# AlexIoannides/bodywork-mlops-demo

Measured on NVIDIA H100. Metric: train rows/sec (N x 128 least-squares fit), higher is better.
Workload: dtype bf16x2 (hi+lo) MMA operands, f32 accumulate, f64 fold+solve

## Files before the change

### bodywork-mlops-demo_b200/csrc/b2_api.cu

```cuda
#include <dlfcn.h>
#include <math.h>
#include <stdarg.h>
#include <stdlib.h>

#include <new>
#include <thread>
#include <vector>

#include "b2_internal.cuh"
#include "b2_xchg.cuh"

namespace b2 {

static thread_local char g_err[768] = "";

void set_error(const char* fmt, ...) {
  va_list ap;
  va_start(ap, fmt);
  vsnprintf(g_err, sizeof(g_err), fmt, ap);
  va_end(ap);
}

namespace {

// ... 242 lines not shown
      },
      [&](int buf, int64_t, int64_t rows) {
        return gram_dispatch(ctx, ctx->stage_x[buf], x_dtype, ctx->stage_y[buf], rows, d, d,
                             mask != nullptr ? ctx->stage_m[buf] : nullptr, keep);
      });
}

int ensure_s_cleared(b2_ctx* ctx) {
  if (ctx->s_zero_pending) {
    B2_CUDA(cudaMemsetAsync(ctx->S, 0, sizeof(double) * kMaxS * kMaxS, ctx->stream));
    ctx->s_zero_pending = false;
  }
  return B2_OK;
}

}

}

using namespace b2;

extern "C" {

int b2_abi_version(void) { return B2_ABI_VERSION; }
const char* b2_last_error(void) { return g_err; }

int b2_device_count(int* n_out) {
  if (n_out == nullptr) { set_error("n_out is null"); return B2_E_ARG; }
  int n = 0;
  cudaError_t e = cudaGetDeviceCount(&n);
  if (e != cudaSuccess) {
    cudaGetLastError();
    *n_out = 0;
    set_error("cudaGetDeviceCount: %s", cudaGetErrorString(e));
    return B2_E_CUDA;
  }
  *n_out = n;
  return B2_OK;
}

static int ctx_allocate(b2_ctx* ctx) {
  B2_CUDA(cudaStreamCreateWithFlags(&ctx->stream, cudaStreamNonBlocking));
  B2_CUDA(cudaStreamCreateWithFlags(&ctx->copy_stream, cudaStreamNonBlocking));
  B2_CUDA(cudaEventCreate(&ctx->ev_t0));
  B2_CUDA(cudaEventCreate(&ctx->ev_t1));
  for (int i = 0; i < kKernelEventPairs; ++i) {
    B2_CUDA(cudaEventCreate(&ctx->ev_k[i][0]));
    B2_CUDA(cudaEventCreate(&ctx->ev_k[i][1]));
  }
  ctx->simt_ctas = ctx->sm_count;
  ctx->score_ctas = ctx->sm_count * 8;
  B2_CUDA(cudaMalloc(reinterpret_cast<void**>(&ctx->S), sizeof(double) * kMaxS * kMaxS));
  B2_CUDA(cudaMalloc(reinterpret_cast<void**>(&ctx->tc_part),
                     sizeof(double) * (size_t)ctx->sm_count * (kTcAccElems + kTcSums)));
  B2_CUDA(cudaMalloc(reinterpret_cast<void**>(&ctx->tc_red), sizeof(double) * (kTcAccElems + 16)));
  B2_CUDA(cudaMalloc(reinterpret_cast<void**>(&ctx->shift), gram_shift_bytes()));
  B2_CUDA(cudaMalloc(reinterpret_cast<void**>(&ctx->simt_part), sizeof(double) * (size_t)ctx->simt_ctas * kMaxS * kMaxS));
  B2_CUDA(cudaMalloc(reinterpret_cast<void**>(&ctx->score_part), sizeof(double) * ((size_t)ctx->score_ctas + 2) * kNStats));
  B2_CUDA(cudaMalloc(reinterpret_cast<void**>(&ctx->coef_dev), sizeof(double) * (kMaxD + 1)));
  B2_CUDA(cudaMalloc(reinterpret_cast<void**>(&ctx->grad_part), sizeof(double) * (size_t)ctx->score_ctas * kGradOut));
  B2_CUDA(cudaMalloc(reinterpret_cast<void**>(&ctx->refine), sizeof(double) * kRfDoubles));
  B2_CUDA(cudaMalloc(reinterpret_cast<void**>(&ctx->loo), sizeof(double) * kLooDoubles));
  B2_CUDA(cudaMalloc(reinterpret_cast<void**>(&ctx->loo_part), sizeof(double) * (size_t)ctx->sm_count * kMaxAlphas));
  B2_CUDA(cudaMalloc(reinterpret_cast<void**>(&ctx->solve_out), sizeof(double) * (2 * kMaxD + 8)));
  B2_CUDA(cudaHostAlloc(reinterpret_cast<void**>(&ctx->solve_host), sizeof(double) * (2 * kMaxD + 8), cudaHostAllocDefault));
  B2_CUDA(cudaMalloc(reinterpret_cast<void**>(&ctx->tc_sync), 64));
  B2_CUDA(cudaMemset(ctx->tc_sync, 0, 64));
  B2_CUDA(cudaHostAlloc(reinterpret_cast<void**>(&ctx->xchg_status_host), 64, cudaHostAllocDefault));
  ctx->xchg_status_host[0] = 0u;
  B2_CUDA(cudaHostAlloc(reinterpret_cast<void**>(&ctx->coef_host), 2 * sizeof(double) * (kMaxD + 1), cudaHostAllocDefault));
  for (int b = 0; b < 2; ++b) B2_CUDA(cudaEventCreateWithFlags(&ctx->ev_coef[b], cudaEventDisableTiming));
  B2_CUDA(cudaMemset(ctx->shift, 0, gram_shift_bytes()));
  B2_CUDA(cudaMemset(ctx->S, 0, sizeof(double) * kMaxS * kMaxS));
  B2_CUDA(cudaMemset(ctx->tc_red, 0, sizeof(double) * (kTcAccElems + 16)));
  return B2_OK;
}

int b2_ctx_create(int device, b2_ctx** out) {
  if (out == nullptr) { set_error("out is null"); return B2_E_ARG; }
  *out = nullptr;
  int n = 0;
  if (b2_device_count(&n) != B2_OK || n == 0) {
    set_error("no usable CUDA device (libb2gram has no CPU fallback)");
    return B2_E_CUDA;
  }
  if (device < 0 || device >= n) { set_error("device %d out of range (0..%d)", device, n - 1); return B2_E_ARG; }
  B2_CUDA(cudaSetDevice(device));
  cudaDeviceProp prop;
  B2_CUDA(cudaGetDeviceProperties(&prop, device));
  if (prop.major != 9 || prop.minor != 0) {
    set_error("device %d is sm_%d%d; libb2gram is built for sm_90a (H100) only", device, prop.major, prop.minor);
    return B2_E_UNSUPPORTED;
  }
  b2_ctx* ctx = new (std::nothrow) b2_ctx();
  if (ctx == nullptr) { set_error("out of host memory"); return B2_E_STATE; }
  ctx->device = device;
  ctx->sm_count = prop.multiProcessorCount;
  ctx->hbm_bytes = prop.totalGlobalMem;
  snprintf(ctx->name, sizeof(ctx->name), "%s", prop.name);
  if (int r = ctx_allocate(ctx)) {
    b2_ctx_destroy(ctx);
    return r;
  }
  *out = ctx;
  return B2_OK;
}

// ... 1157 lines not shown
```

### bodywork-mlops-demo_b200/csrc/b2_internal.cuh

```cuda
#pragma once
#include <cuda.h>
#include <cuda_bf16.h>
#include <cuda_runtime.h>
#include <stdint.h>
#include <stdio.h>
#include <string.h>

#include <type_traits>

#include "../../include/b2gram.h"

namespace b2 {

constexpr int kMaxD = B2_MAX_D;
constexpr int kMaxS = kMaxD + 2;
constexpr int kKernelEventPairs = 64;
constexpr int kMaxRanks = 8;
constexpr size_t kXchgSlotDoubles = (size_t)kMaxS * kMaxS;
constexpr size_t kXchgDataDoubles = 2 * kMaxRanks * kXchgSlotDoubles;
constexpr size_t kXchgBytes = kXchgDataDoubles * sizeof(double) + 256;

constexpr int kTcRows = 64;
constexpr int kTcM = 128;
constexpr int kTcEMax = 16;
inline int tc_e_width(int pack) { return pack >= 3 ? 16 : 8; }
constexpr int kTcTri = kTcM * (kTcM + 1) / 2;
__host__ __device__ constexpr int tc_part_index(int acc, int i, int j, int ew) {
  return acc == 0 ? (j < kTcM ? j * (j + 1) / 2 + i : kTcTri + (j - kTcM) * kTcM + i)
                  : kTcTri + ew * kTcM + j * kTcM + i;
}
__host__ __device__ constexpr int tc_part_elems(int ew, bool d2) {
  return kTcTri + ew * kTcM + (d2 ? (kTcM + ew) * kTcM : 0);
}
constexpr int kTcAccElems = tc_part_elems(kTcEMax, true);
constexpr int kTcSums = 3;

constexpr int kNStats = 10;
constexpr int kGradOut = kMaxD + 1;
constexpr int kRfBeta = 0;
constexpr int kRfB0 = kMaxD;
constexpr int kRfMean = kMaxD + 1;
constexpr int kRfPrevBeta = 2 * kMaxD + 1;
constexpr int kRfPrevB0 = 3 * kMaxD + 1;
constexpr int kRfStep = 3 * kMaxD + 2;
constexpr int kRfGrad = 3 * kMaxD + 3;
constexpr int kRfDoubles = kRfGrad + kGradOut;
constexpr int kOutRefineStep = 2 * kMaxD + 3;
constexpr int kOutRefineGuard = 2 * kMaxD + 4;

constexpr int kMaxAlphas = B2_MAX_ALPHAS;
constexpr int kLooQ = 0;
constexpr int kLooLam = kMaxD * kMaxD;
constexpr int kLooMean = kLooLam + kMaxD;
constexpr int kLooC = kLooMean + kMaxD;
constexpr int kLooMisc = kLooC + kMaxD;
constexpr int kLooAlpha = kLooMisc + 8;
constexpr int kLooCw = kLooAlpha + kMaxAlphas;
constexpr int kLooW = kLooCw + kMaxD * kMaxAlphas;
constexpr int kLooSum = kLooW + kMaxD * kMaxAlphas;
constexpr int kLooDoubles = kLooSum + kMaxAlphas;

struct EnetArgs {
  double l1_ratio, eps, tol;
  int n_alphas, grid, max_iter, positive, fit_intercept;
  double* alphas;
  const double* coef_init;
  double *coefs, *intercepts, *gaps, *iters, *tol_out;
  const double* folds = nullptr;
  const double* l1_ratios = nullptr;
  int n_folds = 1, n_l1 = 1;
  double* mse = nullptr;
};

constexpr int kMaxFolds = 254;
int launch_fold_ranges(b2_ctx* ctx, const uint8_t* fold_of_row, int64_t n, int n_folds, unsigned long long* range);
int launch_fold_sum(b2_ctx* ctx, const double* folds, int n_folds, int d, double* S);

inline int narrow_dp(int d) { return d <= 1 ? 1 : d <= 2 ? 2 : d <= 4 ? 4 : d <= 8 ? 8 : 16; }

void set_error(const char* fmt, ...);

#define B2_CUDA(call)                                                                      \
  do {                                                                                     \
    cudaError_t e_ = (call);                                                               \
    if (e_ != cudaSuccess) {                                                               \
      b2::set_error("%s failed: %s (%s:%d)", #call, cudaGetErrorString(e_), __FILE__, __LINE__); \
      return B2_E_CUDA;                                                                    \
    }                                                                                      \
  } while (0)

}

struct b2_ctx {
  int device = 0;
  int sm_count = 0;
  size_t hbm_bytes = 0;
  char name[128] = {0};
  cudaStream_t stream = nullptr;
  cudaStream_t copy_stream = nullptr;
  cudaEvent_t ev_t0 = nullptr, ev_t1 = nullptr;
  cudaEvent_t ev_k[b2::kKernelEventPairs][2];
  int k_pairs = 0;
  int64_t launches = 0;

  int kernel_mode = B2_KERNEL_AUTO;
  int drain_rows = 8192;
  int precision = B2_PRECISION_SPLIT;

  int d = 0;
  double* S = nullptr;

  double* tc_part = nullptr;
  double* tc_red = nullptr;
  float* shift = nullptr;
  bool solve_attr_set = false;
  double* solve_host = nullptr;
  struct TmCache {
    const void* X = nullptr; const float* y = nullptr; const uint8_t* mask = nullptr;
    int64_t n = 0, ldx = 0; int d = 0, x_dtype = -1;
    int y_map_2d = 0, m_map_2d = 0;
    alignas(64) unsigned char tmX[128], tmY[128], tmM[128];
  } tm_cache;
  double* simt_part = nullptr;
  int simt_ctas = 0;
  double* score_part = nullptr;
  int score_ctas = 0;
  double* coef_dev = nullptr;
  double* grad_part = nullptr;
  double* refine = nullptr;
  double* loo = nullptr;
  double* loo_part = nullptr;
  double* cv_stage[2] = {nullptr, nullptr};
  int cv_stage_alphas = 0;
  double* enet = nullptr;
  size_t enet_doubles = 0;
  double* folds = nullptr;
  size_t folds_doubles = 0;
  int n_folds = 0;
  int folds_d = 0;
  unsigned long long* fold_range = nullptr;
  double* coef_host = nullptr;
  cudaEvent_t ev_coef[2] = {nullptr, nullptr};
  int coef_slot = 0;
  long long* synth_count = nullptr;
  double* solve_out = nullptr;
  void* stage_x[2] = {nullptr, nullptr};
  float* stage_y[2] = {nullptr, nullptr};
  uint8_t* stage_m[2] = {nullptr, nullptr};
  size_t stage_bytes_x = 0;
  int64_t stage_rows = 0;
  cudaEvent_t ev_copied[2] = {nullptr, nullptr};
  cudaEvent_t ev_consumed[2] = {nullptr, nullptr};
  bool ev_consumed_valid[2] = {false, false};
  float* yhat_stage[2] = {nullptr, nullptr};
  void* bounce[2] = {nullptr, nullptr};
  cudaEvent_t ev_bounce[2] = {nullptr, nullptr};
  bool s_zero_pending = false;
  void* comm = nullptr;
  int n_ranks = 1, rank = 0;
  double* xchg = nullptr;
  double* xchg_peer[8] = {nullptr};
  bool p2p_ready = false;
  bool p2p_local = false;
  unsigned int xchg_epoch = 0;
  unsigned long long xchg_timeout_ns = 10000000000ull;
  bool xchg_pending = false;
  unsigned int* xchg_status_host = nullptr;
  unsigned int* tc_sync = nullptr;
// ... 78 lines not shown
```

### bodywork-mlops-demo_b200/csrc/gram_tc.cu

```cuda
#include <cuda_bf16.h>
#include <stdlib.h>

#include "b2_internal.cuh"
#include "b2_ptx.cuh"
#include "b2_shift.cuh"
#include "b2_xchg.cuh"

namespace b2 {
namespace {

constexpr int kConsumerWGs = 2;
constexpr int kXformWarps = 8;
constexpr int kThreads = 128 * (kConsumerWGs + 2);
constexpr int kFirstXformWarp = 4 * kConsumerWGs;
constexpr int kTmaWarp = kFirstXformWarp;
constexpr int kEWarp = kFirstXformWarp + 1;
static_assert(kFirstXformWarp + kXformWarps == kThreads / 32, "warp roles");
constexpr int kProducers = kXformWarps;
constexpr int kConsumerWarps = 4 * kConsumerWGs;
constexpr int kKGroups = kTcRows / 8;
constexpr uint32_t kRawStageBytes = kTcRows * kMaxD * 4;
constexpr uint32_t kOpSBO = 128;
constexpr uint32_t kOpLBO = (16 + 2 + 16) * kOpSBO;
constexpr uint32_t kOpEOff = 16 * kOpSBO;
// ... 142 lines not shown
      "%16, %17, %18, %19, %20, %21, %22, %23, %24, %25, %26, %27, %28, %29, %30, %31, "
      "%32, %33, %34, %35, %36, %37, %38, %39, %40, %41, %42, %43, %44, %45, %46, %47, "
      "%48, %49, %50, %51, %52, %53, %54, %55, %56, %57, %58, %59, %60, %61, %62, %63}, "
      "%64, %65, p, 1, 1, 0, 1;\n\t}"
      : B2_ACC8(0), B2_ACC8(8), B2_ACC8(16), B2_ACC8(24), B2_ACC8(32), B2_ACC8(40), B2_ACC8(48), B2_ACC8(56)
      : "l"(adesc), "l"(bdesc), "r"(scale_d));
}
#undef B2_ACC8
#undef B2_ACC4
constexpr uint32_t kRawBoxBytes = kTcRows * 64 * 2;
__device__ __forceinline__ uint64_t make_raw_desc(uint32_t addr) {
  return (uint64_t)((addr & 0x3FFFFu) >> 4) | ((uint64_t)(kRawBoxBytes >> 4) << 16) | ((uint64_t)(1024u >> 4) << 32) |
         (1ull << 62);
}

__device__ __forceinline__ void st_shared_v4(uint32_t addr, const uint32_t (&v)[4]) {
  asm volatile("st.shared.v4.b32 [%0], {%1, %2, %3, %4};" ::"r"(addr), "r"(v[0]), "r"(v[1]), "r"(v[2]), "r"(v[3])
               : "memory");
}
__device__ __forceinline__ uint32_t lane_id() {
  uint32_t l;
  asm volatile("mov.u32 %0, %%laneid;" : "=r"(l));
  return l;
}
__device__ __forceinline__ void st_shared_f64(uint32_t addr, double v) {
  asm volatile("st.shared.f64 [%0], %1;" ::"r"(addr), "d"(v) : "memory");
}
__device__ __forceinline__ double ld_shared_f64(uint32_t addr) {
  double v;
  asm volatile("ld.shared.f64 %0, [%1];" : "=d"(v) : "r"(addr) : "memory");
  return v;
}
__device__ __forceinline__ void put_f64(double* p, double v, bool add, bool on) {
  if (add)
    asm volatile("{\n\t.reg .pred p;\n\tsetp.ne.b32 p, %2, 0;\n\t@p red.global.add.f64 [%0], %1;\n\t}"
                 ::"l"(p), "d"(v), "r"((uint32_t)on) : "memory");
  else
    asm volatile("{\n\t.reg .pred p;\n\tsetp.ne.b32 p, %2, 0;\n\t@p st.global.f64 [%0], %1;\n\t}"
                 ::"l"(p), "d"(v), "r"((uint32_t)on) : "memory");
}
__device__ __forceinline__ void st_shared_u16(uint32_t addr, uint32_t v) {
  asm volatile("st.shared.u16 [%0], %1;" ::"r"(addr), "h"((unsigned short)v) : "memory");
}
__device__ __forceinline__ void split2(float v0, float v1, uint32_t& hi, uint32_t& lo) {
  const __nv_bfloat162 h = __floats2bfloat162_rn(v0, v1);
  hi = *reinterpret_cast<const uint32_t*>(&h);
  const float h0 = __uint_as_float(hi << 16), h1 = __uint_as_float(hi & 0xffff0000u);
  const __nv_bfloat162 l = __floats2bfloat162_rn(v0 - h0, v1 - h1);
  lo = *reinterpret_cast<const uint32_t*>(&l);
}

constexpr int kRedElems = kTcAccElems + kTcSums;

__device__ __forceinline__ void tc_reduce_range(const double* part, int n_ctas, int n_acc, double* red, int e0, int e1,
                                                double* quarter) {
  const int epb = blockDim.x >> 2;
  const int e = threadIdx.x % epb, q = threadIdx.x / epb;
  const int per = (n_ctas + 3) / 4;
  const int c0 = q * per, c1 = (c0 + per < n_ctas) ? c0 + per : n_ctas;
  for (int base = e0; base < e1; base += epb) {
    const int idx = base + e;
    const bool sum = idx >= n_acc;
    if (idx < e1) {
      const double* src = sum ? part + (size_t)n_ctas * kTcAccElems + (idx - n_acc) : part + idx;
      const size_t stride = sum ? kTcSums : kTcAccElems;
      double acc[8] = {0.0, 0.0, 0.0, 0.0, 0.0, 0.0, 0.0, 0.0};
      int c = c0;
      for (; c + 8 <= c1; c += 8) {
#pragma unroll
        for (int u = 0; u < 8; ++u) acc[u] += __ldcg(src + (size_t)(c + u) * stride);
      }
      for (; c < c1; ++c) acc[0] += __ldcg(src + (size_t)c * stride);
      quarter[q * epb + e] = ((acc[0] + acc[1]) + (acc[2] + acc[3])) + ((acc[4] + acc[5]) + (acc[6] + acc[7]));
    }
    __syncthreads();
    if (q == 0 && idx < e1)
      red[sum ? kTcAccElems + (idx - n_acc) : idx] =
          ((quarter[e] + quarter[epb + e]) + quarter[2 * epb + e]) + quarter[3 * epb + e];
    __syncthreads();
  }
}

__device__ __forceinline__ void grid_barrier(unsigned int* ctr) {
  __syncthreads();
  if (threadIdx.x == 0) {
    __threadfence();
    atomicAdd(ctr, 1u);
    const uint64_t t0 = globaltimer_ns();
    unsigned int seen;
    do {
      asm volatile("ld.acquire.gpu.global.u32 %0, [%1];" : "=r"(seen) : "l"(ctr) : "memory");
      if (seen < gridDim.x) {
        __nanosleep(40);
        if (globaltimer_ns() - t0 > 4000000000ull) __trap();
      }
    } while (seen < gridDim.x);
    __threadfence();
  }
  __syncthreads();
}

__device__ __forceinline__ double tc_fold_value(const double* red, const double* c, int d, int pack, int ew, bool d2,
                                                int idx) {
  const int dp = d + 2;
  const int a = min(idx / dp, idx % dp), b = max(idx / dp, idx % dp);
  auto P = [&](int acc, int i, int j) { return __ldcg(red + tc_part_index(acc, i, j, ew)); };
  auto s1 = [&](int i) {
    double t = 0.0;
    for (int blk = 0; blk < pack; ++blk) {
      const int r = blk * d + i, e = kTcM + 3 * blk;
      t += d2 ? P(0, r, e) + P(1, r, e) : P(0, r, e);
    }
    return t;
  };
  auto sxy = [&](int i) {
    double t = 0.0;
    for (int blk = 0; blk < pack; ++blk) {
      const int r = blk * d + i, e = kTcM + 3 * blk;
      t += d2 ? P(0, r, e + 1) + P(0, r, e + 2) + P(1, r, e + 1) + P(1, r, e + 2) : P(0, r, e + 1) + P(0, r, e + 2);
    }
    return t;
  };
  auto G = [&](int i, int j) {
    double g = 0.0;
    for (int blk = 0; blk < pack; ++blk) {
      const int ia = blk * d + i, ib = blk * d + j;
// ... 21 lines not shown
  using G = TcGeo<RAWB>;
  constexpr int kRawStages = G::kRawStages, kOpStages = G::kOpStages;
  constexpr uint32_t kOffRaw = G::kOffRaw, kOffOp = G::kOffOp, kOffY = G::kOffY, kOffMask = G::kOffMask;
  const int d = DFIX ? DFIX : d_arg;
  extern __shared__ uint8_t smem_raw[];
  const uint32_t sbase = (smem_u32(smem_raw) + 1023u) & ~1023u;
  uint8_t* smem = smem_raw + (sbase - smem_u32(smem_raw));
  const int warp = threadIdx.x >> 5;
  const int lane = threadIdx.x & 31;

  const uint32_t bar_raw_full = sbase + G::kOffBar;
  const uint32_t bar_raw_empty = bar_raw_full + 8 * kRawStages;
  const uint32_t bar_op_full = bar_raw_empty + 8 * kRawStages;
  const uint32_t bar_op_empty = bar_op_full + 8 * kOpStages;
  float* shift_s = reinterpret_cast<float*>(smem + G::kOffShift);

  const int64_t total_tiles = (n_rows + kTcRows - 1) / kTcRows;
  const int64_t tile_begin = (int64_t)blockIdx.x * total_tiles / gridDim.x;
  const int64_t tile_end = (int64_t)(blockIdx.x + 1) * total_tiles / gridDim.x;
  const int my_tiles = (int)(tile_end - tile_begin);

  if (threadIdx.x == 0) {
    for (int s = 0; s < kRawStages; ++s) {
      mbar_init(bar_raw_full + 8 * s, 1);
      mbar_init(bar_raw_empty + 8 * s, kProducers + (RAWB ? kConsumerWarps : 0));
    }
    for (int s = 0; s < kOpStages; ++s) {
      mbar_init(bar_op_full + 8 * s, kProducers);
      mbar_init(bar_op_empty + 8 * s, kConsumerWarps);
    }
    asm volatile("fence.mbarrier_init.release.cluster;" ::: "memory");
  }
  if (warp == kTmaWarp && lane == 0) {
    tma_prefetch_desc(&tmX);
    tma_prefetch_desc(&tmY);
    if (has_mask) tma_prefetch_desc(&tmM);
  }
  for (uint32_t o = threadIdx.x * 16; o < kOpStages * kOpStageBytes; o += kThreads * 16)
    *reinterpret_cast<uint4*>(smem + kOffOp + o) = make_uint4(0, 0, 0, 0);
  for (int j = threadIdx.x; j <= kMaxD; j += kThreads)
    shift_s[j] = j == kMaxD ? shift[kMaxD] : (j < pack * d_orig ? shift[j % d_orig] : 0.f);
  fence_proxy_async_smem();
  __syncthreads();

  if (warp < kConsumerWarps) {
    asm volatile("setmaxnreg.inc.sync.aligned.u32 %0;" ::"n"(G::kConsumerRegs));
    auto consume = [&](auto wg_c) {
      constexpr int WG = decltype(wg_c)::value;
      constexpr int kF1 = kTcM - 64 * WG;
      constexpr int kF2 = RAWB ? kF1 : kTcM;
      constexpr int kC1 = 64 * WG;
      constexpr int kR1 = (kF1 + EW) / 2, kR2 = (kF2 + EW) / 2;
      float acc1[kR1], acc2[kR2];
      double* my_part = part + (size_t)blockIdx.x * kTcAccElems;
      auto store = [&](auto n_regs, int dst_acc, int col0, bool add, auto val) {
        const int ln = (int)lane_id(), row0 = 64 * WG + 16 * (warp & 3) + (ln >> 2);
#pragma unroll
        for (int r = 0; r < decltype(n_regs)::value; ++r) {
          const int col = col0 + 8 * (r >> 2) + 2 * (ln & 3) + (r & 1), h = (r >> 1) & 1, i = row0 + 8 * h;
          const bool lower = dst_acc == 0 && col < kTcM && i > col;
          put_f64(my_part + tc_part_index(dst_acc, i, col, EW), val(r, col, h), add, !lower);
        }
      };
      auto drain = [&](const auto& acc, int dst_acc, int col0, bool add) {
        constexpr int kR = sizeof(acc) / sizeof(float);
        if constexpr (RAWB) {
          constexpr int kF = 2 * kR - EW;
          const double s1[2] = {(double)__shfl_sync(0xffffffffu, acc[kF / 2], lane & ~3),
                                (double)__shfl_sync(0xffffffffu, acc[kF / 2 + 2], lane & ~3)};
          store(std::integral_constant<int, kR>{}, dst_acc, col0, add, [&](int r, int col, int h) {
            return col < kTcM ? (double)acc[r] - (double)shift_s[col] * s1[h] : (double)acc[r];
          });
        } else {
          store(std::integral_constant<int, kR>{}, dst_acc, col0, add, [&](int r, int, int) { return (double)acc[r]; });
        }
      };
      auto release = [&](int tile) {
        mbar_arrive(bar_op_empty + 8 * (tile % kOpStages));
        if constexpr (RAWB) mbar_arrive(bar_raw_empty + 8 * (tile % kRawStages));
      };
      constexpr uint32_t a_off = (uint32_t)WG * 8 * kOpSBO;
      int os = 0, held = -1, in_chunk = 0;
      uint32_t oph = 0;
      bool first_chunk = true;
      for (int it = 0; it < my_tiles; ++it) {
        mbar_wait(bar_op_full + 8 * os, oph, wait_ns);
        const uint32_t op_addr = sbase + kOffOp + os * kOpStageBytes;
        wgmma_fence();
#pragma unroll
        for (int k2 = 0; k2 < kTcRows / 16; ++k2) {
          const uint32_t k_addr = op_addr + k2 * 2 * kOpLBO;
          const uint64_t hi_desc = make_smem_desc(k_addr + a_off), lo_desc = make_smem_desc(k_addr + kOpLoOff + a_off);
          const uint32_t sc1 = (in_chunk > 0 || k2 > 0) ? 1u : 0u, sc2 = (it > 0 || k2 > 0) ? 1u : 0u;
          if constexpr (RAWB) {
            const uint64_t x_desc = make_raw_desc(sbase + kOffRaw + (uint32_t)(it % kRawStages) * kRawStageBytes +
                                                  (uint32_t)WG * kRawBoxBytes + k2 * 16 * 128);
            const uint64_t e_desc = make_smem_desc(k_addr + kOpEOff);
            if (!(dbg & 2u)) {
              wgmma<kF1, 1>(acc1, hi_desc, x_desc, sc1);
              wgmma<EW, 0>(acc1 + kF1 / 2, hi_desc, e_desc, sc1);
            }
            if (SPLIT && !(dbg & 3u)) {
              wgmma<kF2, 1>(acc2, lo_desc, x_desc, sc2);
              wgmma<EW, 0>(acc2 + kF2 / 2, lo_desc, e_desc, sc2);
            }
          } else {
            if (!(dbg & 2u)) wgmma<kF1 + EW, 0>(acc1, hi_desc, make_smem_desc(k_addr + a_off), sc1);
            if (SPLIT && !(dbg & 3u)) wgmma<kF2 + EW, 0>(acc2, lo_desc, make_smem_desc(k_addr), sc2);
          }
        }
        wgmma_commit();
        const bool last = (in_chunk == chunk_tiles - 1) || (it == my_tiles - 1);
        if (last) {
          wgmma_wait<0>();
          fence_regs(acc1);
          if constexpr (SPLIT) fence_regs(acc2);
        } else {
          wgmma_wait<1>();
        }
        if (lane == 0) {
          if (held >= 0) release(held);
          if (last) release(it);
        }
        held = last ? -1 : it;
        if (last) {
          drain(acc1, 0, kC1, !first_chunk);
          first_chunk = false;
          in_chunk = 0;
        } else {
          ++in_chunk;
        }
        if (++os == kOpStages) { os = 0; oph ^= 1; }
      }
      wgmma_wait<0>();
      if constexpr (SPLIT) {
        fence_regs(acc2);
        drain(acc2, RAWB ? 0 : 1, RAWB ? kC1 : 0, RAWB);
      }
    };
    if (__shfl_sync(0xffffffffu, warp, 0) >= 4) consume(std::integral_constant<int, 1>{});
    else consume(std::integral_constant<int, 0>{});
  } else {
    asm volatile("setmaxnreg.dec.sync.aligned.u32 %0;" ::"n"(G::kProducerRegs));
    const uint32_t tx = (uint32_t)(kTcRows * d * sizeof(T)) + kTcRows * pack * 4 + (has_mask ? kTcRows * pack : 0);
    auto issue = [&](int j) {
      const int s = j % kRawStages;
      mbar_wait(bar_raw_empty + 8 * s, ((uint32_t)(j / kRawStages) & 1u) ^ 1u, wait_ns);
      const uint32_t full = bar_raw_full + 8 * s;
      mbar_expect_tx(full, tx);
      const int64_t row0 = (tile_begin + j) * kTcRows;
      tma_load_2d(sbase + kOffRaw + s * kRawStageBytes, &tmX, 0, (int)row0, full);
      if constexpr (RAWB) tma_load_2d(sbase + kOffRaw + s * kRawStageBytes + kRawBoxBytes, &tmX, 64, (int)row0, full);
      const int sub0 = (int)row0 * pack;
      if (y_map_2d) tma_load_2d(sbase + kOffY + s * kYStageBytes, &tmY, 0, sub0 >> 2, full);
      else tma_load_1d(sbase + kOffY + s * kYStageBytes, &tmY, sub0, full);
      if (has_mask == 2) tma_load_2d(sbase + kOffMask + s * kMStageBytes, &tmM, 0, sub0 >> 4, full);
      else if (has_mask) tma_load_1d(sbase + kOffMask + s * kMStageBytes, &tmM, sub0, full);
    };
    const bool issuer = warp == kTmaWarp && lane == 0;
    if (issuer)
      for (int j = 0; j < G::kAhead && j < my_tiles; ++j) issue(j);

    const int t = warp - kFirstXformWarp;
    const int nb = (d + 63) >> 6;
    const int i = 64 * (t % nb) + 2 * lane;
    const uint32_t swp = ((uint32_t)lane >> 2) & 1u;
    const uint32_t st_off = (uint32_t)((i >> 3) * kOpSBO + (i & 7) * 16);
    auto esum = [&]() { return sbase + G::kOffESum + 8 * lane_id(); };
    if (warp == kEWarp) { st_shared_f64(esum(), 0.0); st_shared_f64(esum() + 256, 0.0); st_shared_f64(esum() + 512, 0.0); }
    int rs = 0, os = 0;
    uint32_t rph = 0, oph = 0;
    for (int it = 0; it < my_tiles; ++it) {
      if (issuer && it + G::kAhead < my_tiles) issue(it + G::kAhead);
      __syncwarp();
      mbar_wait(bar_raw_full + 8 * rs, rph, wait_ns);
      mbar_wait(bar_op_empty + 8 * os, oph ^ 1, wait_ns);
      const int64_t row0 = (tile_begin + it) * kTcRows;
      const int64_t left = n_rows - row0;
      const int rows_valid = left < kTcRows ? (int)left : kTcRows;
      const bool full_tile = (!has_mask) && (rows_valid == kTcRows);
      const uint32_t raw_addr = sbase + kOffRaw + rs * kRawStageBytes;
      const uint32_t m_addr = sbase + kOffMask + rs * kMStageBytes;
      const uint32_t op_addr = sbase + kOffOp + os * kOpStageBytes;
      if (warp == kEWarp && !(dbg & 192u)) {
        const uint32_t y_addr = sbase + kOffY + rs * kYStageBytes;
        const uint32_t e_addr = op_addr + kOpEOff;
        const float c_y = shift_s[kMaxD];
        float a = 0.f, b = 0.f, c = 0.f;
        for (int half = 0; half < kTcRows / 32; ++half) {
          const int rr = lane + 32 * half;
// ... 50 lines not shown
              if (use && has_mask) use = (ld_shared_u8(m_addr + (r0 + k) * pack + blk) == (uint32_t)keep);
              if (!use) { v0[k] = 0.f; v1[k] = 0.f; }
            }
          }
          uint32_t h0[4], l0[4], h1[4], l1[4];
#pragma unroll
          for (int p = 0; p < 4; ++p) {
            if constexpr (SPLIT) {
              split2(v0[2 * p], v0[2 * p + 1], h0[p], l0[p]);
              split2(v1[2 * p], v1[2 * p + 1], h1[p], l1[p]);
            } else {
              const __nv_bfloat162 e0 = __floats2bfloat162_rn(v0[2 * p], v0[2 * p + 1]);
              const __nv_bfloat162 e1 = __floats2bfloat162_rn(v1[2 * p], v1[2 * p + 1]);
              h0[p] = *reinterpret_cast<const uint32_t*>(&e0);
              h1[p] = *reinterpret_cast<const uint32_t*>(&e1);
              l0[p] = l1[p] = 0u;
            }
          }
          if (!(dbg & 4u)) {
            const uint32_t dst = op_addr + (uint32_t)g * kOpLBO + st_off;
            uint32_t f[4], s[4];
#pragma unroll
            for (int p = 0; p < 4; ++p) { f[p] = swp ? h1[p] : h0[p]; s[p] = swp ? h0[p] : h1[p]; }
            st_shared_v4(dst + 16 * swp, f);
            st_shared_v4(dst + 16 - 16 * swp, s);
            if constexpr (SPLIT) {
#pragma unroll
              for (int p = 0; p < 4; ++p) { f[p] = swp ? l1[p] : l0[p]; s[p] = swp ? l0[p] : l1[p]; }
              st_shared_v4(dst + kOpLoOff + 16 * swp, f);
              st_shared_v4(dst + kOpLoOff + 16 - 16 * swp, s);
            }
          }
        }
      }
      if (!(dbg & 32u)) fence_proxy_async_smem();
      __syncwarp();
      if (lane == 0) {
        mbar_arrive(bar_op_full + 8 * os);
        mbar_arrive(bar_raw_empty + 8 * rs);
      }
      if (++rs == kRawStages) { rs = 0; rph ^= 1; }
      if (++os == kOpStages) { os = 0; oph ^= 1; }
    }
    if (warp == kEWarp) {
      const uint32_t es = esum();
      double sy = ld_shared_f64(es), syy = ld_shared_f64(es + 256), cnt = ld_shared_f64(es + 512);
#pragma unroll
      for (int o = 16; o > 0; o >>= 1) {
        sy += __shfl_xor_sync(0xffffffffu, sy, o);
        syy += __shfl_xor_sync(0xffffffffu, syy, o);
        cnt += __shfl_xor_sync(0xffffffffu, cnt, o);
      }
      if (lane == 0) {
        double* ys = part + (size_t)gridDim.x * kTcAccElems + kTcSums * blockIdx.x;
        ys[0] = sy; ys[1] = syy; ys[2] = cnt;
      }
    }
  }
}

struct TcFinal {
  int assign;
  int n_ranks, rank;
  unsigned int epoch;
  PeerPtrs peers;
};

constexpr int kFinalizeThreads = 1024;
constexpr int kFinalizeCtas = (kRedElems + kFinalizeThreads / 4 - 1) / (kFinalizeThreads / 4);

__global__ void __launch_bounds__(kFinalizeThreads, 1)
tc_finalize_kernel(const double* part, int n_ctas, double* red, const float* __restrict__ shift, int d, int pack,
                   int ew, int d2, double* S, unsigned int* sync, const TcFinal fin) {
  __shared__ double quarter[kFinalizeThreads];
  __shared__ double c_s[kMaxD + 1];
  for (int j = threadIdx.x; j <= kMaxD; j += blockDim.x) c_s[j] = (double)shift[j];
  {
    constexpr int epb = kFinalizeThreads / 4;
    const int n_acc = tc_part_elems(ew, d2 != 0);
    const int n_red = n_acc + kTcSums;
    const int per = (((n_red + (int)gridDim.x - 1) / (int)gridDim.x) + epb - 1) / epb * epb;
    const int e0 = (int)blockIdx.x * per;
    const int e1 = e0 + per < n_red ? e0 + per : n_red;
    if (e0 < n_red) tc_reduce_range(part, n_ctas, n_acc, red, e0, e1, quarter);
  }
  grid_barrier(sync + 0);
  {
    const int dp = d + 2;
    const int total = dp * dp;
    const size_t slot = xchg_slot_offset(fin.epoch, fin.rank);
    for (int idx = (int)(blockIdx.x * blockDim.x + threadIdx.x); idx < total; idx += (int)(gridDim.x * blockDim.x)) {
      const double val = tc_fold_value(red, c_s, d, pack, ew, d2 != 0, idx);
      const double sv = fin.assign ? val : S[idx] + val;
      S[idx] = sv;
      if (fin.n_ranks > 1) xchg_store_all(fin.peers, fin.n_ranks, slot, idx, sv);
    }
    if (fin.n_ranks > 1) __threadfence_system();
  }
  __syncthreads();
  __shared__ bool last_cta;
  if (threadIdx.x == 0) {
    __threadfence();
    last_cta = (atomicAdd(sync + 2, 1u) == gridDim.x - 1);
    if (last_cta) {
      sync[0] = 0u; sync[2] = 0u;
      __threadfence();
    }
  }
  __syncthreads();
  if (last_cta && fin.n_ranks > 1) xchg_publish(fin.peers, fin.n_ranks, fin.rank, fin.epoch);
}

typedef CUresult (*PFN_encodeTiled)(CUtensorMap*, CUtensorMapDataType, cuuint32_t, void*, const cuuint64_t*,
                                    const cuuint64_t*, const cuuint32_t*, const cuuint32_t*, CUtensorMapInterleave,
                                    CUtensorMapSwizzle, CUtensorMapL2promotion, CUtensorMapFloatOOBfill);

PFN_encodeTiled get_encode() {
  static PFN_encodeTiled fn = nullptr;
  if (fn == nullptr) {
    void* p = nullptr;
    cudaDriverEntryPointQueryResult q;
    if (cudaGetDriverEntryPoint("cuTensorMapEncodeTiled", &p, cudaEnableDefault, &q) == cudaSuccess &&
        q == cudaDriverEntryPointSuccess)
      fn = reinterpret_cast<PFN_encodeTiled>(p);
  }
  return fn;
}

}

bool gram_tc_supported(const void* X, int x_dtype, const float* y, int64_t n, int d, int64_t ldx,
                       const uint8_t* mask) {
  const int es = x_dtype == B2_F32 ? 4 : 2;
  if (d < 4 || d > kMaxD) return false;
  if ((d * es) % 16 != 0) return false;
  if ((ldx * es) % 16 != 0) return false;
  if ((reinterpret_cast<uintptr_t>(X) & 15) != 0 || (reinterpret_cast<uintptr_t>(y) & 15) != 0) return false;
// ... 90 lines not shown
  } else {
    int y_map_2d = 0, m_map_2d = 0;
    if (int r = encode_maps(encode, X, x_dtype, es, y, n, d_tensor, d, ldx, n_y, pack, mask, rawb, &tmX, &tmY, &tmM, &y_map_2d,
                            &m_map_2d))
      return r;
    tc.X = X; tc.y = y; tc.mask = mask; tc.n = n_in; tc.ldx = ldx_in; tc.d = d_in; tc.x_dtype = x_dtype;
    tc.y_map_2d = y_map_2d; tc.m_map_2d = m_map_2d;
    memcpy(tc.tmX, &tmX, sizeof(tmX)); memcpy(tc.tmY, &tmY, sizeof(tmY)); memcpy(tc.tmM, &tmM, sizeof(tmM));
  }

  const int64_t total_tiles = (n + kTcRows - 1) / kTcRows;
  const int sms = (ctx->sm_limit > 0 && ctx->sm_limit < ctx->sm_count) ? ctx->sm_limit : ctx->sm_count;
  const int grid = (int)(total_tiles < sms ? total_tiles : sms);
  int chunk_tiles = ctx->drain_rows / kTcRows / (rawb ? 4 : 1);
  if (chunk_tiles < 1) chunk_tiles = 1;

#ifdef B2_DEV_KNOBS
  static const uint32_t wait_ns = []() {
    const char* e = getenv("B2_WAIT_HINT_NS");
    return e ? (uint32_t)atoi(e) : 20000u;
  }();
#else
  constexpr uint32_t wait_ns = 20000u;
#endif
#ifdef B2_DEV_KNOBS
  static const uint32_t dbg = []() {
    const char* e = getenv("B2_TC_DEBUG");
    return e ? (uint32_t)atoi(e) : 0u;
  }();
#else
  constexpr uint32_t dbg = 0u;
#endif
  const bool split = ctx->precision == B2_PRECISION_SPLIT;
  const int ew = tc_e_width(pack);
  const bool d2 = split && !rawb;
  decltype(&gram_tc_kernel<float, 0, false>) kernel = nullptr;
  uint32_t smem = TcGeo<false>::kSmemBytes;
  with_rows(x_dtype, X, [&](auto* Xr) {
    using T = row_t<decltype(Xr)>;
    return with_int<0, 1>(split, [&](auto SP) {
      constexpr bool kSplit = decltype(SP)::value;
      if (d != 128) kernel = gram_tc_kernel<T, 0, kSplit>;
      else if (ew == 16) kernel = gram_tc_kernel<T, 128, kSplit, false, 16>;
      else kernel = gram_tc_kernel<T, 128, kSplit>;
      if constexpr (std::is_same_v<T, __nv_bfloat16>) {
        if (rawb) {
          kernel = gram_tc_kernel<T, 128, kSplit, true>;
          smem = TcGeo<true>::kSmemBytes;
        }
      }
      return B2_OK;
    });
  });
  B2_CUDA(cudaFuncSetAttribute(kernel, cudaFuncAttributeMaxDynamicSharedMemorySize, smem));
  const int pair = ctx->k_pairs % kKernelEventPairs;
  B2_CUDA(cudaEventRecord(ctx->ev_k[pair][0], ctx->stream));
  kernel<<<grid, kThreads, smem, ctx->stream>>>(tmX, tmY, tmM, tc.y_map_2d, mask != nullptr ? 1 + tc.m_map_2d : 0, keep,
                                                n, d, pack, d_in, ctx->shift, chunk_tiles, ctx->tc_part, wait_ns, dbg);
  B2_CUDA(cudaGetLastError());
  B2_CUDA(cudaEventRecord(ctx->ev_k[pair][1], ctx->stream));
  ctx->k_pairs += 1;

  TcFinal fin;
  memset(&fin, 0, sizeof(fin));
  fin.assign = assign ? 1 : 0;
  fin.n_ranks = 1;
  if (scatter_epoch != 0) {
    fin.n_ranks = ctx->n_ranks; fin.rank = ctx->rank; fin.epoch = scatter_epoch;
    for (int r = 0; r < kMaxRanks; ++r) fin.peers.p[r] = ctx->xchg_peer[r];
  }
  {
    cudaLaunchConfig_t cfg;
    memset(&cfg, 0, sizeof(cfg));
    cfg.gridDim = dim3(kFinalizeCtas < sms ? kFinalizeCtas : sms);
    cfg.blockDim = dim3(kFinalizeThreads); cfg.dynamicSmemBytes = 0; cfg.stream = ctx->stream;
    cudaLaunchAttribute attr[1];
    attr[0].id = cudaLaunchAttributeCooperative;
    attr[0].val.cooperative = 1;
    cfg.attrs = attr; cfg.numAttrs = 1;
    const double* part_arg = ctx->tc_part;
    const float* shift_arg = ctx->shift;
    B2_CUDA(cudaLaunchKernelEx(&cfg, tc_finalize_kernel, part_arg, grid, ctx->tc_red, shift_arg, d_in, pack, ew,
                               d2 ? 1 : 0, ctx->S, ctx->tc_sync, fin));
  }
  ctx->launches += 2;
  return B2_OK;
}

}
```

### bodywork-mlops-demo_b200/csrc/solve.cu

```cuda
#include "b2_internal.cuh"
#include "b2_xchg.cuh"

namespace b2 {
namespace {

constexpr int kOutIntercept = kMaxD;
constexpr int kOutInfo = kMaxD + 1;
constexpr int kOutRank = kMaxD + 2;
constexpr int kOutSingular = kMaxD + 3;
constexpr int kOutRows = kOutSingular + kMaxD;

struct LdcgStat {
  const double* S;
  __device__ __forceinline__ double operator()(int i) const { return __ldcg(S + i); }
};

template <class Stat>
__device__ void build_normal_equations_of(const Stat& S, int d, double alpha, int fit_intercept,
                                       double* A, double* r, double* mean, double* ybar_out) {
  const int dp = d + 2, pitch = d + 1;
  const double n = S(d * dp + d);
  const double inv_n = n > 0.0 ? 1.0 / n : 0.0;
  double sxy = 0.0;
  if ((int)threadIdx.x < d) {
// ... 2 lines not shown
    mean[threadIdx.x] = fit_intercept ? sx * inv_n : 0.0;
  }
  const double ybar = fit_intercept ? S(d * dp + d + 1) * inv_n : 0.0;
  __syncthreads();
  if ((int)threadIdx.x < d) r[threadIdx.x] = sxy - n * mean[threadIdx.x] * ybar;
  const int lane = threadIdx.x & 31, warp = threadIdx.x >> 5, nwarps = blockDim.x >> 5;
  for (int i0 = warp; i0 < d; i0 += 2 * nwarps) {
    const int i1 = i0 + nwarps;
    double v[8];
#pragma unroll
    for (int u = 0; u < 4; ++u) {
      const int j = lane + 32 * u;
      v[u] = j < d ? S(i0 * dp + j) : 0.0;
      v[4 + u] = (j < d && i1 < d) ? S(i1 * dp + j) : 0.0;
    }
    const double m0 = mean[i0], m1 = i1 < d ? mean[i1] : 0.0;
#pragma unroll
    for (int u = 0; u < 4; ++u) {
      const int j = lane + 32 * u;
      if (j < d) {
        const double mj = mean[j];
        A[i0 * pitch + j] = v[u] - n * m0 * mj + (i0 == j ? alpha : 0.0);
        if (i1 < d) A[i1 * pitch + j] = v[4 + u] - n * m1 * mj + (i1 == j ? alpha : 0.0);
      }
    }
  }
  if (threadIdx.x == 0) *ybar_out = ybar;
  __syncthreads();
}

__device__ __forceinline__ void build_normal_equations(const double* S, int d, double alpha, int fit_intercept,
                                                       double* A, double* r, double* mean, double* ybar_out) {
  build_normal_equations_of(LdcgStat{S}, d, alpha, fit_intercept, A, r, mean, ybar_out);
}

__device__ __forceinline__ double rcp_pos(double x) {
  double y;
  asm("rcp.approx.ftz.f64 %0, %1;" : "=d"(y) : "d"(x));
  const double er = fma(-x, y, 1.0);
  const double t = fma(er, er, er);
  return fma(y, t, y);
}

struct SolveXchg {
  double* own;
  int n_ranks;
  unsigned int epoch;
  unsigned long long timeout_ns;
};

constexpr int kNB = 16;
constexpr int kCholThreads = 512;
constexpr int kUPitch = kNB + 1;

__device__ void refine_update(const double* S, int d, int fit_intercept, bool singular, const double* dbeta, double* misc,
                              double* __restrict__ rf, double* __restrict__ out);

template <bool REFINE>
__global__ void __launch_bounds__(kCholThreads, 1)
solve_cholesky_kernel(double* S, int d, double alpha, int fit_intercept, double* __restrict__ out, const SolveXchg xc,
                      double* __restrict__ rf) {
  extern __shared__ double sm[];
  const int pitch = d + 1;
  double* A = sm;
  double* r = A + d * pitch;
  double* mean = A + (d + 1) * pitch;
  double* invd = mean + d;
  double* misc = invd + d;
  double* U = misc + 8;
  const int tid = threadIdx.x, lane = tid & 31;
  const int warp = __shfl_sync(0xffffffffu, tid >> 5, 0);
  long long tm[5] = {0, 0, 0, 0, 0};
  long long tc0 = clock64();
  if (xc.own != nullptr) {
    __shared__ int ok;
    if (tid == 0) ok = xchg_wait(xc.own, xc.n_ranks, xc.epoch, xc.timeout_ns) ? 1 : 0;
    __syncthreads();
    if (!ok) {
      if (tid == 0) {
        xchg_flags(xc.own)[kXchgStatusWord] = xc.epoch;
        out[kOutInfo] = -1.0;
      }
      return;
    }
    const int dp = d + 2;
    for (int base = 0; base < dp * dp; base += 4 * blockDim.x) {
      double sv[4];
#pragma unroll
      for (int u = 0; u < 4; ++u) {
        const int idx = base + u * blockDim.x + tid;
        sv[u] = idx < dp * dp ? xchg_sum(xc.own, xc.n_ranks, xc.epoch, idx) : 0.0;
      }
#pragma unroll
      for (int u = 0; u < 4; ++u) {
        const int idx = base + u * blockDim.x + tid;
        if (idx < dp * dp) S[idx] = sv[u];
      }
    }
    __threadfence();
    __syncthreads();
  }
  build_normal_equations(S, d, alpha, fit_intercept, A, r, mean, &misc[0]);
  if constexpr (REFINE) {
    if (tid < d) r[tid] = rf[kRfGrad + tid] - alpha * rf[kRfBeta + tid];
    __syncthreads();
  }
  tm[0] = clock64() - tc0;
  if (warp == 0) {
    double mx = 0.0;
    for (int i = lane; i < d; i += 32) mx = fmax(mx, A[i * pitch + i]);
#pragma unroll
    for (int o = 16; o > 0; o >>= 1) mx = fmax(mx, __shfl_xor_sync(0xffffffffu, mx, o));
    if (lane == 0) { misc[1] = mx; misc[2] = 0.0; }
  }
  __syncthreads();
  const double tiny = misc[1] * 1e-12;
  const int rows = d + 1;

  for (int kb = 0; kb < d; kb += kNB) {
    const int nb = (d - kb) < kNB ? (d - kb) : kNB;
    tc0 = clock64();
    if (warp == 0) {
      const int lrow = lane & (kNB - 1), h = lane >> 4;
      const bool act = lrow < nb;
      const int row = kb + (act ? lrow : 0);
      double a[kNB / 2];
// ... 43 lines not shown
      double sv[4];
#pragma unroll
      for (int j = 0; j < 4; ++j) {
        const int c = 4 * j + q;
        sv[j] = (live && c < nb) ? A[i * pitch + kb + c] : 0.0;
      }
      const int qbase = lane & ~3;
      double rinv[kNB];
#pragma unroll
      for (int m = 0; m < kNB; ++m) rinv[m] = m < nb ? invd[kb + m] : 0.0;
      double out_m[4], out_u[4];
#pragma unroll
      for (int j = 0; j < 4; ++j) { out_m[j] = 0.0; out_u[j] = 0.0; }
#pragma unroll
      for (int m = 0; m < kNB; ++m) {
        if (m < nb) {
          const double um = __shfl_sync(0xffffffffu, sv[m >> 2], qbase | (m & 3));
          const double xm = um * rinv[m];
          if (q == (m & 3)) { out_m[m >> 2] = xm; out_u[m >> 2] = um; }
#pragma unroll
          for (int j = 0; j < 4; ++j) {
            if (4 * j + 3 > m) {
              const int c = 4 * j + q;
              if (c > m && c < nb) sv[j] = fma(-xm, U[(kb + c) * kUPitch + m], sv[j]);
            }
          }
        }
      }
      if (live) {
#pragma unroll
        for (int j = 0; j < 4; ++j) {
          const int m = 4 * j + q;
          if (m < nb) { A[i * pitch + kb + m] = out_m[j]; U[i * kUPitch + m] = out_u[j]; }
        }
      }
    }
    __syncthreads();
    tm[2] += clock64() - tc0; tc0 = clock64();
    {
      const int base = kb + nb;
      const int nti = (rows - base + 7) >> 3, ntj = (d - base + 7) >> 3;
      const int tri = ntj * (ntj + 1) / 2;
      const int total = tri + (nti > ntj ? ntj : 0);
      const int g = lane >> 2, t4 = lane & 3;
      constexpr int kWarps = kCholThreads / 32, kInFlight = 4;
      for (int t0 = warp; t0 < total; t0 += kWarps * kInFlight) {
        int ia[kInFlight], jb[kInFlight];
        double c0[kInFlight], c1[kInFlight], av[kInFlight][kNB / 4], bv[kInFlight][kNB / 4];
#pragma unroll
        for (int f = 0; f < kInFlight; ++f) {
          const int t = t0 + f * kWarps;
          int ti = 0, tj = 0;
          if (t < tri) {
            ti = (int)((sqrtf(8.0f * (float)t + 1.0f) - 1.0f) * 0.5f);
            while (ti * (ti + 1) / 2 > t) --ti;
            while ((ti + 1) * (ti + 2) / 2 <= t) ++ti;
            tj = t - ti * (ti + 1) / 2;
          } else if (t < total) {
            ti = ntj; tj = t - tri;
          }
          const bool live = t < total;
          ia[f] = live ? base + 8 * ti + g : rows;
          jb[f] = live ? base + 8 * tj + g : d;
#pragma unroll
          for (int sgm = 0; sgm < kNB / 4; ++sgm) {
            const int m = 4 * sgm + t4;
            av[f][sgm] = (ia[f] < rows && m < nb) ? -A[ia[f] * pitch + kb + m] : 0.0;
            bv[f][sgm] = (jb[f] < d && m < nb) ? U[jb[f] * kUPitch + m] : 0.0;
          }
          c0[f] = 0.0; c1[f] = 0.0;
        }
#pragma unroll
        for (int sgm = 0; sgm < kNB / 4; ++sgm) {
#pragma unroll
          for (int f = 0; f < kInFlight; ++f)
            asm volatile("mma.sync.aligned.m8n8k4.row.col.f64.f64.f64.f64 {%0, %1}, {%2}, {%3}, {%0, %1};"
                         : "+d"(c0[f]), "+d"(c1[f]) : "d"(av[f][sgm]), "d"(bv[f][sgm]));
        }
#pragma unroll
        for (int f = 0; f < kInFlight; ++f) {
          const int jc = jb[f] - g + 2 * t4;
          if (ia[f] < rows) {
            if (jc < d) A[ia[f] * pitch + jc] += c0[f];
            if (jc + 1 < d) A[ia[f] * pitch + jc + 1] += c1[f];
          }
        }
      }
    }
    __syncthreads();
    tm[3] += clock64() - tc0;
  }
  tc0 = clock64();
  const bool singular = misc[2] != 0.0;
  if (!singular) {
    for (int kb = ((d - 1) / kNB) * kNB; kb >= 0; kb -= kNB) {
      const int nb = (d - kb) < kNB ? (d - kb) : kNB;
      if (warp == 0) {
        const int col = lane & (kNB - 1);
        const bool act = lane < nb;
        double lt[kNB];
#pragma unroll
        for (int k = 0; k < kNB; ++k) lt[k] = (act && k < nb && k > col) ? A[(kb + k) * pitch + kb + col] : 0.0;
        double z = act ? r[kb + col] : 0.0;
#pragma unroll
        for (int k = kNB - 1; k >= 0; --k) {
          if (k < nb) {
            const double bk = __shfl_sync(0xffffffffu, z, k);
            z = (lane < k) ? fma(-lt[k], bk, z) : z;
          }
        }
// ... 1017 lines not shown
```

Measured before the change: 5.444 billion.

## Store split-precision second accumulator as f32 partials, cache smem attributes, tabulate tiles

The non-raw split path now writes the second (correction) accumulator into per-CTA partials as f32 instead of f64. This halves its partial storage and shrinks the per-CTA stride, and the cross-CTA reduction reads those floats and widens them to double while summing. The change also skips repeated cudaFuncSetAttribute calls by remembering which kernels already have their shared-memory size set. The Cholesky solve now builds a shared lookup table of triangular tile indices once, replacing the per-tile sqrt and loop computation. Storing the low-order correction terms in f32 could slightly reduce accuracy.

```diff
diff --git a/bodywork-mlops-demo_b200/csrc/b2_api.cu b/bodywork-mlops-demo_b200/csrc/b2_api.cu
--- a/bodywork-mlops-demo_b200/csrc/b2_api.cu
+++ b/bodywork-mlops-demo_b200/csrc/b2_api.cu
@@ -318,7 +318,7 @@
   ctx->score_ctas = ctx->sm_count * 8;
   B2_CUDA(cudaMalloc(reinterpret_cast<void**>(&ctx->S), sizeof(double) * kMaxS * kMaxS));
   B2_CUDA(cudaMalloc(reinterpret_cast<void**>(&ctx->tc_part),
-                     sizeof(double) * (size_t)ctx->sm_count * (kTcAccElems + kTcSums)));
+                     sizeof(double) * (size_t)ctx->sm_count * (kTcPartStride + kTcSums)));
   B2_CUDA(cudaMalloc(reinterpret_cast<void**>(&ctx->tc_red), sizeof(double) * (kTcAccElems + 16)));
   B2_CUDA(cudaMalloc(reinterpret_cast<void**>(&ctx->shift), gram_shift_bytes()));
   B2_CUDA(cudaMalloc(reinterpret_cast<void**>(&ctx->simt_part), sizeof(double) * (size_t)ctx->simt_ctas * kMaxS * kMaxS));
diff --git a/bodywork-mlops-demo_b200/csrc/b2_internal.cuh b/bodywork-mlops-demo_b200/csrc/b2_internal.cuh
--- a/bodywork-mlops-demo_b200/csrc/b2_internal.cuh
+++ b/bodywork-mlops-demo_b200/csrc/b2_internal.cuh
@@ -29,11 +29,14 @@
   return acc == 0 ? (j < kTcM ? j * (j + 1) / 2 + i : kTcTri + (j - kTcM) * kTcM + i)
                   : kTcTri + ew * kTcM + j * kTcM + i;
 }
+__host__ __device__ constexpr int tc_d1_elems(int ew) { return kTcTri + ew * kTcM; }
 __host__ __device__ constexpr int tc_part_elems(int ew, bool d2) {
-  return kTcTri + ew * kTcM + (d2 ? (kTcM + ew) * kTcM : 0);
+  return tc_d1_elems(ew) + (d2 ? (kTcM + ew) * kTcM : 0);
 }
 constexpr int kTcAccElems = tc_part_elems(kTcEMax, true);
+constexpr int kTcPartStride = tc_d1_elems(kTcEMax) + (kTcM + kTcEMax) * kTcM / 2;
 constexpr int kTcSums = 3;
+constexpr int kTcKernels = 14;
 
 constexpr int kNStats = 10;
 constexpr int kGradOut = kMaxD + 1;
@@ -114,6 +117,7 @@
   double* tc_red = nullptr;
   float* shift = nullptr;
   bool solve_attr_set = false;
+  const void* tc_attr_set[b2::kTcKernels] = {nullptr};
   double* solve_host = nullptr;
   struct TmCache {
     const void* X = nullptr; const float* y = nullptr; const uint8_t* mask = nullptr;
diff --git a/bodywork-mlops-demo_b200/csrc/gram_tc.cu b/bodywork-mlops-demo_b200/csrc/gram_tc.cu
--- a/bodywork-mlops-demo_b200/csrc/gram_tc.cu
+++ b/bodywork-mlops-demo_b200/csrc/gram_tc.cu
@@ -218,8 +218,27 @@
 
 constexpr int kRedElems = kTcAccElems + kTcSums;
 
-__device__ __forceinline__ void tc_reduce_range(const double* part, int n_ctas, int n_acc, double* red, int e0, int e1,
-                                                double* quarter) {
+template <typename V>
+__device__ __forceinline__ double tc_sum_ctas(const V* src, size_t stride, int c0, int c1) {
+  double acc[8] = {0.0, 0.0, 0.0, 0.0, 0.0, 0.0, 0.0, 0.0};
+  int c = c0;
+  for (; c + 16 <= c1; c += 16) {
+    V v[16];
+#pragma unroll
+    for (int u = 0; u < 16; ++u) v[u] = __ldcg(src + (size_t)(c + u) * stride);
+#pragma unroll
+    for (int u = 0; u < 16; ++u) acc[u & 7] += (double)v[u];
+  }
+  for (; c + 8 <= c1; c += 8) {
+#pragma unroll
+    for (int u = 0; u < 8; ++u) acc[u] += (double)__ldcg(src + (size_t)(c + u) * stride);
+  }
+  for (; c < c1; ++c) acc[0] += (double)__ldcg(src + (size_t)c * stride);
+  return ((acc[0] + acc[1]) + (acc[2] + acc[3])) + ((acc[4] + acc[5]) + (acc[6] + acc[7]));
+}
+
+__device__ __forceinline__ void tc_reduce_range(const double* part, int n_ctas, int n_d1, int n_acc, double* red, int e0,
+                                                int e1, double* quarter) {
   const int epb = blockDim.x >> 2;
   const int e = threadIdx.x % epb, q = threadIdx.x / epb;
   const int per = (n_ctas + 3) / 4;
@@ -228,16 +247,12 @@
     const int idx = base + e;
     const bool sum = idx >= n_acc;
     if (idx < e1) {
-      const double* src = sum ? part + (size_t)n_ctas * kTcAccElems + (idx - n_acc) : part + idx;
-      const size_t stride = sum ? kTcSums : kTcAccElems;
-      double acc[8] = {0.0, 0.0, 0.0, 0.0, 0.0, 0.0, 0.0, 0.0};
-      int c = c0;
-      for (; c + 8 <= c1; c += 8) {
-#pragma unroll
-        for (int u = 0; u < 8; ++u) acc[u] += __ldcg(src + (size_t)(c + u) * stride);
-      }
-      for (; c < c1; ++c) acc[0] += __ldcg(src + (size_t)c * stride);
-      quarter[q * epb + e] = ((acc[0] + acc[1]) + (acc[2] + acc[3])) + ((acc[4] + acc[5]) + (acc[6] + acc[7]));
+      double v;
+      if (sum) v = tc_sum_ctas(part + (size_t)n_ctas * kTcPartStride + (idx - n_acc), kTcSums, c0, c1);
+      else if (idx >= n_d1)
+        v = tc_sum_ctas(reinterpret_cast<const float*>(part + n_d1) + (idx - n_d1), 2 * (size_t)kTcPartStride, c0, c1);
+      else v = tc_sum_ctas(part + idx, kTcPartStride, c0, c1);
+      quarter[q * epb + e] = v;
     }
     __syncthreads();
     if (q == 0 && idx < e1)
@@ -365,7 +380,7 @@
       constexpr int kC1 = 64 * WG;
       constexpr int kR1 = (kF1 + EW) / 2, kR2 = (kF2 + EW) / 2;
       float acc1[kR1], acc2[kR2];
-      double* my_part = part + (size_t)blockIdx.x * kTcAccElems;
+      double* my_part = part + (size_t)blockIdx.x * kTcPartStride;
       auto store = [&](auto n_regs, int dst_acc, int col0, bool add, auto val) {
         const int ln = (int)lane_id(), row0 = 64 * WG + 16 * (warp & 3) + (ln >> 2);
 #pragma unroll
@@ -448,7 +463,17 @@
       wgmma_wait<0>();
       if constexpr (SPLIT) {
         fence_regs(acc2);
-        drain(acc2, RAWB ? 0 : 1, RAWB ? kC1 : 0, RAWB);
+        if constexpr (RAWB) {
+          drain(acc2, 0, kC1, true);
+        } else {
+          float* d2 = reinterpret_cast<float*>(my_part + tc_d1_elems(EW));
+          const int ln = (int)lane_id(), row0 = 64 * WG + 16 * (warp & 3) + (ln >> 2);
+#pragma unroll
+          for (int r = 0; r < kR2; ++r) {
+            const int col = 8 * (r >> 2) + 2 * (ln & 3) + (r & 1), i = row0 + 8 * ((r >> 1) & 1);
+            d2[tc_part_index(1, i, col, EW) - tc_d1_elems(EW)] = acc2[r];
+          }
+        }
       }
     };
     if (__shfl_sync(0xffffffffu, warp, 0) >= 4) consume(std::integral_constant<int, 1>{});
@@ -605,7 +630,7 @@
         cnt += __shfl_xor_sync(0xffffffffu, cnt, o);
       }
       if (lane == 0) {
-        double* ys = part + (size_t)gridDim.x * kTcAccElems + kTcSums * blockIdx.x;
+        double* ys = part + (size_t)gridDim.x * kTcPartStride + kTcSums * blockIdx.x;
         ys[0] = sy; ys[1] = syy; ys[2] = cnt;
       }
     }
@@ -635,7 +660,7 @@
     const int per = (((n_red + (int)gridDim.x - 1) / (int)gridDim.x) + epb - 1) / epb * epb;
     const int e0 = (int)blockIdx.x * per;
     const int e1 = e0 + per < n_red ? e0 + per : n_red;
-    if (e0 < n_red) tc_reduce_range(part, n_ctas, n_acc, red, e0, e1, quarter);
+    if (e0 < n_red) tc_reduce_range(part, n_ctas, tc_d1_elems(ew), n_acc, red, e0, e1, quarter);
   }
   grid_barrier(sync + 0);
   {
@@ -832,7 +857,15 @@
       return B2_OK;
     });
   });
-  B2_CUDA(cudaFuncSetAttribute(kernel, cudaFuncAttributeMaxDynamicSharedMemorySize, smem));
+  {
+    const void* kfn = reinterpret_cast<const void*>(kernel);
+    int k = 0;
+    while (k < kTcKernels && ctx->tc_attr_set[k] != nullptr && ctx->tc_attr_set[k] != kfn) ++k;
+    if (k == kTcKernels || ctx->tc_attr_set[k] == nullptr) {
+      B2_CUDA(cudaFuncSetAttribute(kernel, cudaFuncAttributeMaxDynamicSharedMemorySize, smem));
+      if (k < kTcKernels) ctx->tc_attr_set[k] = kfn;
+    }
+  }
   const int pair = ctx->k_pairs % kKernelEventPairs;
   B2_CUDA(cudaEventRecord(ctx->ev_k[pair][0], ctx->stream));
   kernel<<<grid, kThreads, smem, ctx->stream>>>(tmX, tmY, tmM, tc.y_map_2d, mask != nullptr ? 1 + tc.m_map_2d : 0, keep,
diff --git a/bodywork-mlops-demo_b200/csrc/solve.cu b/bodywork-mlops-demo_b200/csrc/solve.cu
--- a/bodywork-mlops-demo_b200/csrc/solve.cu
+++ b/bodywork-mlops-demo_b200/csrc/solve.cu
@@ -78,6 +78,7 @@
 constexpr int kNB = 16;
 constexpr int kCholThreads = 512;
 constexpr int kUPitch = kNB + 1;
+constexpr int kTriTiles = (kMaxD / 8) * (kMaxD / 8 + 1) / 2;
 
 __device__ void refine_update(const double* S, int d, int fit_intercept, bool singular, const double* dbeta, double* misc,
                               double* __restrict__ rf, double* __restrict__ out);
@@ -98,6 +99,12 @@
   const int warp = __shfl_sync(0xffffffffu, tid >> 5, 0);
   long long tm[5] = {0, 0, 0, 0, 0};
   long long tc0 = clock64();
+  __shared__ unsigned short tile_ij[kTriTiles];
+  for (int t = tid; t < kTriTiles; t += blockDim.x) {
+    int ti = 0;
+    while ((ti + 1) * (ti + 2) / 2 <= t) ++ti;
+    tile_ij[t] = (unsigned short)(ti | (t - ti * (ti + 1) / 2) << 8);
+  }
   if (xc.own != nullptr) {
     __shared__ int ok;
     if (tid == 0) ok = xchg_wait(xc.own, xc.n_ranks, xc.epoch, xc.timeout_ns) ? 1 : 0;
@@ -247,10 +254,8 @@
           const int t = t0 + f * kWarps;
           int ti = 0, tj = 0;
           if (t < tri) {
-            ti = (int)((sqrtf(8.0f * (float)t + 1.0f) - 1.0f) * 0.5f);
-            while (ti * (ti + 1) / 2 > t) --ti;
-            while ((ti + 1) * (ti + 2) / 2 <= t) ++ti;
-            tj = t - ti * (ti + 1) / 2;
+            const int ij = tile_ij[t];
+            ti = ij & 0xff; tj = ij >> 8;
           } else if (t < total) {
             ti = ntj; tj = t - tri;
           }
```

After: 5.452 billion (median of 6 runs). About the same (+0.2%).
